# mgholamikn/PoseGen

Measured on AMD Instinct MI355X. Metric: rendered rays/sec (512x512, 64 samples/ray), higher is better.
Workload: dtype bf16

## Files before the change

include/posegen_hip.h:

```cpp
#ifndef POSEGEN_HIP_H
#define POSEGEN_HIP_H

#include <stdint.h>

#ifdef __cplusplus
extern "C" {
#endif

#define PG_ABI_VERSION 11

#define PG_OK 0
#define PG_EINVAL (-1)
#define PG_ENOMEM (-2)
#define PG_EHIP (-3)
#define PG_ESTATE (-4)

#define PG_PREC_FP32 0
#define PG_PREC_BF16 1
#define PG_PREC_BF16X3 2
#define PG_PREC_FP16 3
#define PG_PREC_FP16X3 4
#define PG_PREC_FP16C 5
#define PG_PREC_COUNT 6
#define PG_PREC_FP16M 6
// ... 138 lines not shown

int pg_stage_eval(pg_handle* h, void* stream, int which_net, int64_t n, int n_samples,
                  const float* ray_batch, const float* z, const float* skts,
                  int64_t pose_stride, const float* cams, float* raw, float* dbg, int dbg_stage);

int pg_query_density(pg_handle* h, void* stream, int which_net, int64_t n_points, const float* pts,
                     const float* skts, float* raw);

int pg_stage_composite(pg_handle* h, void* stream, int64_t n, int n_samples,
                       const float* ray_batch, const float* z, const float* raw,
                       float* rgb, float* disp, float* acc, float* alpha, float* weights,
                       int n_importance, float* z_fine );

int pg_set_far_skip(pg_handle* h, int on);

int pg_load_weights_device(pg_handle* h, void* stream, int which_net, const float* const* d_tensors, int n_tensors,
                           const float* d_codes, int n_codes);

#define PG_ONCHIP_RECORDS 0
#define PG_ONCHIP_AUTO 1
#define PG_ONCHIP_ALWAYS 2
int pg_set_onchip(pg_handle* h, int mode);

int pg_set_train_precision(pg_handle* h, int precision);

int pg_profile_enable(pg_handle* h, int on);
int pg_profile_read(pg_handle* h, int64_t* n_launches, double* total_ms, int64_t* n_points);
int pg_profile_read_aux(pg_handle* h, int64_t* n_launches, double* total_ms);

int pg_debug_pack(const float* const* tensors, const int64_t* shapes, int n_tensors,
// ... 24 lines not shown
```

posegen_amd/_ffi.py:

```python
from __future__ import annotations

import ctypes as C
import os
from typing import Optional

_HERE = os.path.dirname(os.path.abspath(__file__))
LIB_PATH = os.path.join(_HERE, "_lib", "libposegen_hip.so")

PG_OK, PG_EINVAL, PG_ENOMEM, PG_EHIP, PG_ESTATE = 0, -1, -2, -3, -4
PG_FLAG_LINDISP = 1
PG_ACT_RELU, PG_ACT_SOFTPLUS = 0, 1
PG_ABI_VERSION = 11


class HipLibraryError(RuntimeError):
    """libposegen_hip.so is missing or unusable (no CPU fallback exists)."""


class PgError(RuntimeError):
    def __init__(self, code: int, msg: str):
        super().__init__(f"posegen_hip error {code}: {msg}")
        self.code = code


# ... 26 lines not shown
                                   "alpha0", "near_far", "z_coarse", "z_fine", "raw_coarse", "raw_fine",
                                   "weights0")]


PROTOTYPES = {
    "pg_abi_version": (C.c_int, []),
    "pg_create": (C.c_int, [C.POINTER(PgConfig), C.c_int, C.POINTER(C.c_int), C.POINTER(C.c_void_p)]),
    "pg_destroy": (None, [C.c_void_p]),
    "pg_last_error": (C.c_char_p, [C.c_void_p]),
    "pg_load_weights": (C.c_int, [C.c_void_p, C.c_int, C.POINTER(C.c_void_p), C.POINTER(C.c_int64), C.c_int]),
    "pg_set_embedder": (C.c_int, [C.c_void_p, C.c_int, C.c_void_p, C.c_float]),
    "pg_set_framecodes": (C.c_int, [C.c_void_p, C.c_int, C.c_void_p, C.c_int]),
    "pg_set_precision": (C.c_int, [C.c_void_p, C.c_int]),
    "pg_set_chunk": (C.c_int, [C.c_void_p, C.c_int]),
    "pg_set_far_skip": (C.c_int, [C.c_void_p, C.c_int]),
    "pg_set_onchip": (C.c_int, [C.c_void_p, C.c_int]),
    "pg_load_weights_device": (C.c_int, [C.c_void_p, C.c_void_p, C.c_int, C.POINTER(C.c_void_p), C.c_int, C.c_void_p, C.c_int]),
    "pg_set_train_precision": (C.c_int, [C.c_void_p, C.c_int]),
    "pg_render_rays": (C.c_int, [C.c_void_p, C.c_void_p, C.c_int64, _FP, _FP, C.c_int64, _FP, C.c_int64, _FP,
                                 C.c_int, C.c_int, C.c_int, C.POINTER(PgOutputs)]),
    "pg_calibrate_mfma": (C.c_int, [C.c_void_p, C.c_int, C.c_int, C.c_double, C.POINTER(C.c_double), C.POINTER(C.c_double)]),
    "pg_render_rays_train": (C.c_int, [C.c_void_p, C.c_void_p, C.c_int64, _FP, _FP, C.c_int64, _FP, C.c_int64, _FP,
                                       C.c_int, C.c_int, C.c_int, C.POINTER(PgTrainDraws), C.POINTER(PgOutputs)]),
    "pg_stage_sample_coarse": (C.c_int, [C.c_void_p, C.c_void_p, C.c_int64, _FP, _FP, C.c_int64, C.c_int,
                                         C.c_int, _FP, _FP]),
    "pg_stage_eval": (C.c_int, [C.c_void_p, C.c_void_p, C.c_int, C.c_int64, C.c_int, _FP, _FP, _FP,
                                C.c_int64, _FP, _FP, _FP, C.c_int]),
    "pg_stage_composite": (C.c_int, [C.c_void_p, C.c_void_p, C.c_int64, C.c_int, _FP, _FP, _FP, _FP, _FP, _FP,
                                     _FP, _FP, C.c_int, _FP]),
    "pg_profile_enable": (C.c_int, [C.c_void_p, C.c_int]),
# ... 75 lines not shown
```

posegen_amd/csrc/pg_api.hip:

```cpp
#include <hip/hip_runtime.h>

#include <cstdarg>
#include <cstdio>
#include <cstdlib>
#include <chrono>
#include <cstring>
#include <algorithm>
#include <mutex>
#include <thread>
#include <new>
#include <utility>
#include <vector>

#include "../../include/posegen_hip.h"
#include "pg_device.h"
#include "pg_handle.h"
#include "pg_pack.h"

extern "C" {
int pg_launch_eval16(const pgd::EvalArgs* a, int fp16, int framecode, int grid, void* stream);
int pg_launch_eval16r(const pgd::EvalArgs* a, int fp16, int framecode, int onchip, int grid, void* stream);
int pg_launch_ray_records(const pgd::RecArgs* a, int fp16, int framecode, int n_cu, void* stream);
int pg_eval16_points_per_pass(void);
int pg_eval16_wgs_per_cu(void);
// ... 137 lines not shown
    F_C2,
    F_COMP_DIRECT,
    F_COMP_REC,
    F_COMP_ONCHIP,
    F_KMAJOR,
    F_COUNT
};

constexpr int PASS_WALK_RHO = 99;
struct Switches {
    bool view_fact = true;
    bool comp_kernel = true;
    bool comp_rec = true;
    bool evalc2 = true;
    int onchip = PG_ONCHIP_AUTO;
    int pass_walk = PASS_WALK_RHO;
};
const Switches& switches() {
    static const Switches sw = [] {
        auto off = [](const char* name) { const char* e = std::getenv(name); return e && e[0] == '0'; };
        Switches s;
        s.view_fact = !off("POSEGEN_VIEW_FACT");
        s.comp_kernel = !off("POSEGEN_COMP_KERNEL");
        s.comp_rec = !off("POSEGEN_COMP_REC");
        s.evalc2 = !off("POSEGEN_EVALC2");
        const char* e = std::getenv("POSEGEN_ONCHIP");
        s.onchip = e && e[0] == '0' ? PG_ONCHIP_RECORDS : e && e[0] == '2' ? PG_ONCHIP_ALWAYS : PG_ONCHIP_AUTO;
        if (const char* w = std::getenv("POSEGEN_PASS_WALK")) s.pass_walk = std::max(0, std::atoi(w));
        return s;
    }();
    return sw;
}

struct CallFacts {
    int prec;
    int S;
    long long pose_stride;
    bool fc;
    bool points, pnoise;
    bool dbg; int dbg_stage;
// ... 227 lines not shown
    hipError_t e = hipMalloc(reinterpret_cast<void**>(&h->ws), want);
    if (e != hipSuccess) return pg_fail(h, PG_ENOMEM, "workspace allocation of %zu bytes failed: %s", want, hipGetErrorString(e));
    h->ws_bytes = want;
    return PG_OK;
}

int check_ready(pg_handle* h, bool need_fine) {
    if (!h) return pg_fail(nullptr, PG_EINVAL, "null handle");
    need_fine = need_fine && !h->cfg.single_net;
    if (!h->net[0].loaded) return pg_fail(h, PG_ESTATE, "coarse network weights not loaded (pg_load_weights)");
    if (need_fine && !h->net[1].loaded) return pg_fail(h, PG_ESTATE, "fine network weights not loaded (pg_load_weights)");
    if (!h->emb_set[0] || !h->emb_set[1]) return pg_fail(h, PG_ESTATE, "embedder state not set (pg_set_embedder)");
    return PG_OK;
}

int launch_eval_one(pg_handle* h, void* stream, int which, long long n, int S, const float* rays, const float* z,
                    const float* skts, long long pose_stride, const float* cams, float* raw, float* dbg, int dbg_stage,
                    const float* points, const float* pnoise, bool guide_pass) {
    const int prec = pass_precision(h->cfg.precision, guide_pass);
    const bool fc = h->cfg.framecode_ch > 0;
    const Form form = pick_form(CallFacts{prec, S, pose_stride, fc, points != nullptr, pnoise != nullptr, dbg != nullptr, dbg_stage, h->onchip_mode}, switches());
    const FormInfo& fi = FORMS[form];
    const int y_bytes = fi.rec_y_bytes;
    int rc = ensure_form_images(h, which, form, prec, fc);
    if (rc) return rc;
    if (y_bytes && (rc = ensure_rec(h, n, y_bytes))) return rc;
    NetState& ns = h->net[which];
    if (fc && !ns.d_codes) return pg_fail(h, PG_ESTATE, "frame codes of net %d not set (pg_set_framecodes)", which);
    pgd::EvalArgs a{};
    a.rays = rays; a.z = z; a.pts = points; a.pnoise = pnoise; a.skts = skts; a.cams = cams;
    a.codes = fc ? ns.d_codes : nullptr;
    a.wstream = ns.img[image_of(fi.stream, prec)].d;
    a.wy = fi.wy == IMG_NONE || (fi.wy == IMG_YCODE && !fc) ? nullptr : ns.img[image_of(fi.wy, prec)].d;
    a.bias = reinterpret_cast<const float*>(ns.img[fi.bias].d);
    if (y_bytes) {
        a.rec_y = h->rec;
// ... 4 lines not shown
                                     (size_t)REC_PAD_RAYS * REC_AB_BYTES, static_cast<hipStream_t>(stream)));
            h->rec_pad_n = n; h->rec_pad_y = y_bytes; h->rec_pad_stream = stream;
        }
    }
    a.cutoff = h->d_cut;
    a.raw = raw; a.dbg = dbg;
    a.pose_stride = pose_stride;
    a.n_points = n * S;
    a.n_rays = (int)n;
    a.S = S;
    a.n_codes = ns.n_codes;
    a.tau_v = h->tau[0];
    a.tau_d = h->tau[1];
    a.dbg_stage = dbg_stage;
    a.far_skip = h->far_skip ? 1 : 0;
    const int pts = fi.points_per_pass();
    if (!points && S < pts / (MAXR - 1))
        return pg_fail(h, PG_EINVAL, "N_samples=%d too small: the fused kernel needs >= %d samples per ray", S, pts / (MAXR - 1));
    const long long iters = (a.n_points + pts - 1) / pts;
    a.n_iters = (int)iters;
    static const long long wg_cap = [] { const char* e = std::getenv("POSEGEN_MAX_WG"); return e ? std::atoll(e) : 0ll; }();
    long long max_wg = (long long)h->n_cu * fi.wgs_per_cu();
    if (wg_cap > 0 && wg_cap < max_wg) max_wg = wg_cap;
    const int grid = (int)(iters < max_wg ? iters : max_wg);
    a.walk_rho = switches().pass_walk % grid;
    hipEvent_t e0 = nullptr, e1 = nullptr;
    auto get = [&](hipEvent_t& ev) {
        if (!h->ev_free.empty()) { ev = h->ev_free.back(); h->ev_free.pop_back(); return hipSuccess; }
        return hipEventCreate(&ev);
    };
// ... 28 lines not shown
    case F_COMP_REC:    e = pg_launch_evalc(&a, fc, 1, grid, stream); break;
    case F_COMP_ONCHIP: e = pg_launch_evalc(&a, fc, 2, grid, stream); break;
    default:            e = pg_launch_eval32(&a, prec, fc, grid, stream); break;
    }
    if (h->profiling) {
        PG_HIP(h, hipEventRecord(e1, static_cast<hipStream_t>(stream)));
        h->ev_used.emplace_back(e0, e1);
        h->prof_points += a.n_points;
    }
    if (e) return pg_fail(h, PG_EHIP, "fused embed+MLP kernel launch failed: %s", hipGetErrorString((hipError_t)e));
    return PG_OK;
}

int launch_eval(pg_handle* h, void* stream, int which, long long n, int S, const float* rays, const float* z,
                const float* skts, long long pose_stride, const float* cams, float* raw, float* dbg, int dbg_stage = 0,
                const float* points = nullptr, const float* pnoise = nullptr, bool guide_pass = false) {
    long long batch = 1ll << 19;
    if (const char* e = std::getenv("POSEGEN_REC_BATCH")) { const long long v = std::atoll(e); if (v >= 64) batch = v; }
    if (points || dbg || n <= batch)
        return launch_eval_one(h, stream, which, n, S, rays, z, skts, pose_stride, cams, raw, dbg, dbg_stage, points, pnoise, guide_pass);
    for (long long r0 = 0; r0 < n; r0 += batch) {
        const long long m = std::min(batch, n - r0);
        const int rc = launch_eval_one(h, stream, which, m, S, rays + r0 * 11, z + r0 * S, skts + r0 * pose_stride, pose_stride,
                                       cams ? cams + r0 : nullptr, raw + r0 * S * 4, nullptr, 0, nullptr,
                                       pnoise ? pnoise + r0 * S * 3 : nullptr, guide_pass);
        if (rc) return rc;
    }
    return PG_OK;
}

}

int pg_sc_scratch(pg_handle* h, long long n, int chunk, double** out) {
    *out = nullptr;
    const long long need = pg_sample_coarse_scratch(n, chunk);
    if (need <= 0) return PG_OK;
    if ((size_t)need > h->sc_part_cap) {
        PG_HIP(h, hipSetDevice(h->device));
        if (h->sc_part) { PG_HIP(h, hipDeviceSynchronize()); PG_HIP(h, hipFree(h->sc_part)); h->sc_part = nullptr; h->sc_part_cap = 0; }
        const size_t want = (size_t)need * 2;
// ... 19 lines not shown
    if (cfg->n_joints != J || cfg->multires != LV || (cfg->multires_views != LD && cfg->multires_views != 0) || cfg->multires_bones != 0 ||
        cfg->net_depth != DEPTH || cfg->net_width != W || cfg->skip_layer != SKIP || cfg->view_width != VW ||
        (cfg->framecode_ch != 0 && cfg->framecode_ch != FC_CH))
        return pg_fail(nullptr, PG_EINVAL,
                    "pg_create: unsupported architecture (kernels are built for 24 joints, multires 7/{4,0}/0, "
                    "8x256 trunk, skip 4, view width 128, frame code 0|16)");
    if (cfg->single_net != 0 && cfg->single_net != 1) return pg_fail(nullptr, PG_EINVAL, "pg_create: single_net must be 0 or 1, got %d", cfg->single_net);
    if (cfg->precision < 0 || cfg->precision >= PG_PREC_MODES) return pg_fail(nullptr, PG_EINVAL, "pg_create: bad precision %d", cfg->precision);
    if (is_x3(cfg->precision) && !x3_allowed())
        return pg_fail(nullptr, PG_EINVAL, "pg_create: split-operand precision %d is experimental (set POSEGEN_EXPERIMENTAL_X3=1)", cfg->precision);
    if (cfg->chunk <= 0) return pg_fail(nullptr, PG_EINVAL, "pg_create: chunk must be positive");
    if (!(cfg->density_scale > 0.f)) return pg_fail(nullptr, PG_EINVAL, "pg_create: density_scale must be positive");
    if (cfg->density_act != PG_ACT_RELU && cfg->density_act != PG_ACT_SOFTPLUS)
        return pg_fail(nullptr, PG_EINVAL, "pg_create: density_act must be PG_ACT_RELU or PG_ACT_SOFTPLUS, got %d", cfg->density_act);
    pg_handle* h = new (std::nothrow) pg_handle();
    if (h) h->onchip_mode = switches().onchip;
    if (!h) return pg_fail(nullptr, PG_ENOMEM, "pg_create: out of host memory");
    h->cfg = *cfg;
    h->device = device_ids ? device_ids[0] : 0;
    for (int i = 0; i < 48; ++i) h->cut[i] = cfg->cutoff_dist;
    int ndev = 0;
    hipError_t e = hipGetDeviceCount(&ndev);
    if (e != hipSuccess || ndev <= 0) { delete h; return pg_fail(nullptr, PG_EHIP, "pg_create: no HIP device available (%s)", hipGetErrorString(e)); }
    if (h->device < 0 || h->device >= ndev) { delete h; return pg_fail(nullptr, PG_EINVAL, "pg_create: device %d out of range (%d devices)", cfg ? device_ids ? device_ids[0] : 0 : 0, ndev); }
    hipDeviceProp_t prop;
    if (hipSetDevice(h->device) != hipSuccess || hipGetDeviceProperties(&prop, h->device) != hipSuccess) {
        delete h;
        return pg_fail(nullptr, PG_EHIP, "pg_create: cannot query device");
    }
    h->n_cu = prop.multiProcessorCount > 0 ? prop.multiProcessorCount : 256;
    h->clock_khz = prop.clockRate;
// ... 223 lines not shown
    return PG_OK;
}

int pg_set_chunk(pg_handle* h, int chunk) {
    if (!h) return pg_fail(nullptr, PG_EINVAL, "pg_set_chunk: null handle");
    if (chunk <= 0) return pg_fail(h, PG_EINVAL, "pg_set_chunk: chunk must be positive, got %d", chunk);
    h->cfg.chunk = chunk;
    PG_FORWARD(h, pg_set_chunk(hh, chunk));
    return PG_OK;
}

int pg_set_far_skip(pg_handle* h, int on) {
    if (!h) return pg_fail(nullptr, PG_EINVAL, "pg_set_far_skip: null handle");
    h->far_skip = on != 0;
    PG_FORWARD(h, pg_set_far_skip(hh, on));
    return PG_OK;
}

int pg_set_onchip(pg_handle* h, int mode) {
    if (!h) return pg_fail(nullptr, PG_EINVAL, "pg_set_onchip: null handle");
    if (mode < PG_ONCHIP_RECORDS || mode > PG_ONCHIP_ALWAYS) return pg_fail(h, PG_EINVAL, "pg_set_onchip: mode must be 0 (records), 1 (by sample count) or 2 (on chip), got %d", mode);
    h->onchip_mode = mode;
    PG_FORWARD(h, pg_set_onchip(hh, mode));
    return PG_OK;
}

int pg_set_train_precision(pg_handle* h, int precision) {
    if (!h) return pg_fail(nullptr, PG_EINVAL, "null handle");
    if (precision != PG_PREC_FP32 && precision != PG_PREC_BF16)
        return pg_fail(h, PG_EINVAL, "pg_set_train_precision: the training step computes in fp32 (PG_PREC_FP32) or on a bf16 tape (PG_PREC_BF16), not %d", precision);
// ... 248 lines not shown
    if (e) return pg_fail(h, PG_EHIP, "sample_coarse launch failed: %s", hipGetErrorString((hipError_t)e));
    return PG_OK;
}

int pg_stage_eval(pg_handle* h, void* stream, int which, int64_t n, int n_samples, const float* ray_batch,
                  const float* z, const float* skts, int64_t pose_stride, const float* cams, float* raw, float* dbg,
                  int dbg_stage) {
    int rc = check_ready(h, which == 1);
    if (rc) return rc;
    if (which < 0 || which > 1) return pg_fail(h, PG_EINVAL, "pg_stage_eval: which_net must be 0 or 1");
    if (which == 1 && h->cfg.single_net) return pg_fail(h, PG_EINVAL, "pg_stage_eval: a single_net handle has one net (which_net 0)");
    if (n < 0 || !ray_batch || !z || !skts || !raw) return pg_fail(h, PG_EINVAL, "pg_stage_eval: null/negative argument");
    if (pose_stride != 0 && pose_stride != 384) return pg_fail(h, PG_EINVAL, "pose_stride must be 0 or 384");
    if (n == 0) return PG_OK;
    PG_HIP(h, hipSetDevice(h->device));
    return launch_eval(h, stream, which, n, n_samples, ray_batch, z, skts, pose_stride, cams, raw, dbg, dbg_stage);
}

int pg_query_density(pg_handle* h, void* stream, int which, int64_t n_points, const float* pts, const float* skts,
                     float* raw) {
    int rc = check_ready(h, which == 1);
    if (rc) return rc;
    if (which < 0 || which > 1) return pg_fail(h, PG_EINVAL, "pg_query_density: which_net must be 0 or 1");
    if (which == 1 && h->cfg.single_net) return pg_fail(h, PG_EINVAL, "pg_query_density: a single_net handle has one net (which_net 0)");
    if (n_points < 0 || !pts || !skts || !raw) return pg_fail(h, PG_EINVAL, "pg_query_density: null/negative argument");
    if (n_points > 0x7fffffffLL) return pg_fail(h, PG_EINVAL, "pg_query_density: at most 2^31-1 points per call");
    if (n_points == 0) return PG_OK;
    PG_HIP(h, hipSetDevice(h->device));
    rc = ensure_ws(h, 256);
    if (rc) return rc;
    PG_HIP(h, hipMemsetAsync(h->ws, 0, 64, static_cast<hipStream_t>(stream)));
// ... 67 lines not shown
    int* order = reinterpret_cast<int*>(p); p += b_ord;
    float* zn = reinterpret_cast<float*>(p); p += b_zn;
    float* rawn = reinterpret_cast<float*>(p); p += b_rn;
    float* pn = b_pn ? reinterpret_cast<float*>(p) : nullptr;
    {
        double* scs = nullptr;
        if (int rc2 = pg_sc_scratch(h, n, h->cfg.chunk, &scs)) return rc2;
        int e0 = pg_launch_sample_coarse(ray_batch, cyls, cyl_stride, n, h->cfg.chunk, S, (flags & PG_FLAG_LINDISP) ? 1 : 0, nf, zc,
                                         dr ? dr->t_rand : nullptr, scs, stream);
        if (e0) return pg_fail(h, PG_EHIP, "coarse sampling launch failed: %s", hipGetErrorString((hipError_t)e0));
    }
    if (rnoise) {
        int e0 = pg_launch_gather_noise(dr->ray_noise, n, SF, S, nullptr, pn, stream);
        if (e0) return pg_fail(h, PG_EHIP, "noise gather launch failed: %s", hipGetErrorString((hipError_t)e0));
    }
    rc = launch_eval(h, stream, 0, n, S, ray_batch, zc, skts, pose_stride, cams, rawc, nullptr, 0, nullptr, rnoise ? pn : nullptr, false);
    if (rc) return rc;
    int e = pg_launch_composite_iso(ray_batch, zc, rawc, n, S, h->cfg.density_scale, h->cfg.rgb_eps, h->cfg.density_act,
                                    h->cfg.softplus_shift, out->rgb0, out->disp0, out->acc0, out->alpha0,
                                    out->weights0 ? out->weights0 : w0, N, zf, dr ? dr->noise0 : nullptr, dr ? dr->u_rand : nullptr,
                                    order, zn, NP, stream);
    if (e) return pg_fail(h, PG_EHIP, "composite launch failed: %s", hipGetErrorString((hipError_t)e));
    if (rnoise) {
        e = NP == N ? pg_launch_gather_noise(dr->ray_noise + (size_t)S * 3, n, SF, N, nullptr, pn, stream)
                    : (int)hipMemsetAsync(pn, 0, (size_t)n * NP * 12, s);
        if (!e && NP != N)
            e = (int)hipMemcpy2DAsync(pn, (size_t)NP * 12, dr->ray_noise + (size_t)S * 3, (size_t)SF * 12, (size_t)N * 12, (size_t)n,
                                      hipMemcpyDeviceToDevice, s);
        if (e) return pg_fail(h, PG_EHIP, "noise gather failed: %s", hipGetErrorString((hipError_t)e));
    }
    rc = launch_eval(h, stream, 0, n, NP, ray_batch, zn, skts, pose_stride, cams, rawn, nullptr, 0, nullptr, rnoise ? pn : nullptr, false);
    if (rc) return rc;
    e = pg_launch_composite_merged(ray_batch, zf, rawc, rawn, NP, order, n, S, N, h->cfg.density_scale, h->cfg.rgb_eps, h->cfg.density_act,
                                   h->cfg.softplus_shift, out->rgb_map, out->disp_map, out->acc_map, out->alpha,
                                   dr ? dr->noise1 : nullptr, out->raw_fine, stream);
    if (e) return pg_fail(h, PG_EHIP, "composite launch failed: %s", hipGetErrorString((hipError_t)e));
    if (out->near_far) PG_HIP(h, hipMemcpyAsync(out->near_far, nf, (size_t)n * 8, hipMemcpyDeviceToDevice, s));
    if (out->z_coarse) PG_HIP(h, hipMemcpyAsync(out->z_coarse, zc, (size_t)n * S * 4, hipMemcpyDeviceToDevice, s));
    if (out->raw_coarse) PG_HIP(h, hipMemcpyAsync(out->raw_coarse, rawc, (size_t)n * S * 16, hipMemcpyDeviceToDevice, s));
    if (out->z_fine) PG_HIP(h, hipMemcpyAsync(out->z_fine, zf, (size_t)n * SF * 4, hipMemcpyDeviceToDevice, s));
    return PG_OK;
}

int render_rays_impl(pg_handle* h, void* stream, int64_t n, const float* ray_batch, const float* skts,
                     int64_t pose_stride, const float* cyls, int64_t cyl_stride, const float* cams, int n_samples,
                     int n_importance, int flags, const pg_train_draws* dr, const pg_outputs* out) {
// ... 30 lines not shown
    float* rawf = reinterpret_cast<float*>(p); p += hier ? b_rf : 0;
    int* order = b_ord ? reinterpret_cast<int*>(p) : nullptr; p += b_ord;
    float* pn = b_pn ? reinterpret_cast<float*>(p) : nullptr;

    {
        double* scs = nullptr;
        if (int rc = pg_sc_scratch(h, n, h->cfg.chunk, &scs)) return rc;
        int e0 = pg_launch_sample_coarse(ray_batch, cyls, cyl_stride, n, h->cfg.chunk, S, (flags & PG_FLAG_LINDISP) ? 1 : 0, nf, zc,
                                         dr ? dr->t_rand : nullptr, scs, stream);
        if (e0) return pg_fail(h, PG_EHIP, "coarse sampling launch failed: %s", hipGetErrorString((hipError_t)e0));
    }
    if (rnoise) {
        int e0 = pg_launch_gather_noise(dr->ray_noise, n, SF, S, nullptr, pn, stream);
        if (e0) return pg_fail(h, PG_EHIP, "noise gather launch failed: %s", hipGetErrorString((hipError_t)e0));
    }
    rc = launch_eval(h, stream, 0, n, S, ray_batch, zc, skts, pose_stride, cams, rawc, nullptr, 0, nullptr, rnoise ? pn : nullptr, hier);
    if (rc) return rc;
    int e = pg_launch_composite(ray_batch, zc, rawc, n, S, h->cfg.density_scale, h->cfg.rgb_eps, h->cfg.density_act, h->cfg.softplus_shift,
                                hier ? out->rgb0 : out->rgb_map, hier ? out->disp0 : out->disp_map,
                                hier ? out->acc0 : out->acc_map, hier ? out->alpha0 : out->alpha,
                                out->weights0 ? out->weights0 : w0, n_importance, hier ? zf : nullptr,
                                dr ? dr->noise0 : nullptr, dr ? dr->u_rand : nullptr, order, stream);
    if (e) return pg_fail(h, PG_EHIP, "composite launch failed: %s", hipGetErrorString((hipError_t)e));
    if (hier) {
        if (rnoise) {
            e = pg_launch_gather_noise(dr->ray_noise, n, SF, SF, order, pn, stream);
            if (e) return pg_fail(h, PG_EHIP, "noise gather launch failed: %s", hipGetErrorString((hipError_t)e));
        }
        rc = launch_eval(h, stream, 1, n, SF, ray_batch, zf, skts, pose_stride, cams, rawf, nullptr, 0, nullptr, rnoise ? pn : nullptr);
        if (rc) return rc;
        e = pg_launch_composite(ray_batch, zf, rawf, n, SF, h->cfg.density_scale, h->cfg.rgb_eps, h->cfg.density_act, h->cfg.softplus_shift, out->rgb_map,
                                out->disp_map, out->acc_map, out->alpha, nullptr, 0, nullptr, dr ? dr->noise1 : nullptr,
                                nullptr, nullptr, stream);
        if (e) return pg_fail(h, PG_EHIP, "composite launch failed: %s", hipGetErrorString((hipError_t)e));
    }
    if (out->near_far) PG_HIP(h, hipMemcpyAsync(out->near_far, nf, (size_t)n * 8, hipMemcpyDeviceToDevice, s));
    if (out->z_coarse) PG_HIP(h, hipMemcpyAsync(out->z_coarse, zc, (size_t)n * S * 4, hipMemcpyDeviceToDevice, s));
    if (out->raw_coarse) PG_HIP(h, hipMemcpyAsync(out->raw_coarse, rawc, (size_t)n * S * 16, hipMemcpyDeviceToDevice, s));
    if (hier && out->z_fine) PG_HIP(h, hipMemcpyAsync(out->z_fine, zf, (size_t)n * SF * 4, hipMemcpyDeviceToDevice, s));
    if (hier && out->raw_fine) PG_HIP(h, hipMemcpyAsync(out->raw_fine, rawf, (size_t)n * SF * 16, hipMemcpyDeviceToDevice, s));
    return PG_OK;
}
}

// ... 500 lines not shown
```

posegen_amd/csrc/pg_device.h:

```cpp
#pragma once
#include <hip/hip_runtime.h>

#include <atomic>

#include "pg_program.h"

namespace pgd {
using namespace pgl;

typedef __attribute__((ext_vector_type(8))) __bf16 bf16x8;
typedef __attribute__((ext_vector_type(8))) _Float16 f16x8;
typedef __attribute__((ext_vector_type(16))) float f32x16;

struct EvalArgs {
    const float* rays;
    const float* z;
    const float* pts;
    const float* pnoise;
    const float* skts;
    const float* cams;
    const float* codes;
    const uint8_t* wstream;
    const uint8_t* wy;
    const float* rec_ab;
    const uint8_t* rec_y;
    const float* bias;
    const float* cutoff;
    float* raw;
    float* dbg;
    long long pose_stride;
    long long n_points;
    int n_rays;
    int S;
    int n_codes;
    int n_iters;
    float tau_v, tau_d;
    int dbg_stage;
    int far_skip;
    int walk_rho;
};

struct RecArgs {
    const float* rays;
    const float* skts;
    const float* cams;
    const float* codes;
    const uint8_t* wy;
    float* rec_ab;
    uint8_t* rec_y;
    const float* z;
    long long pose_stride;
    int n_rays;
    int n_codes;
// ... 433 lines not shown
```

posegen_amd/csrc/pg_eval16_common.h:

```cpp
#pragma once
#include "pg_device.h"

namespace pgd {
using namespace pgp::A;

#ifndef PG_A_WAVES
#define PG_A_WAVES 8
#endif
constexpr int NWAVE = PG_A_WAVES;
constexpr int NTHR = NWAVE * 64;
constexpr int PTS = NWAVE * 32;

template <typename V> struct Op;
template <> struct Op<bf16x8> {
    using E = __bf16;
    static __device__ __forceinline__ f32x16 mfma(bf16x8 a, bf16x8 b, f32x16 c) {
#if defined(PG_MFMA_TURNS)
        asm volatile("s_setprio 1\n\tv_mfma_f32_32x32x16_bf16 %0, %1, %2, %0\n\ts_setprio 0" : "+v"(c) : "v"(a), "v"(b));
        return c;
#endif
        return __builtin_amdgcn_mfma_f32_32x32x16_bf16(a, b, c, 0, 0, 0);
    }
    static __device__ __forceinline__ bf16x8 cvt(const float* x) {
        bf16x8 v;
// ... 111 lines not shown
    }
#endif
    if (LA <= rem) st.issue(p.r[(L + LA) % NS], q + LA);
    if (PG_SPREAD_DMA) {
        if (q % PSTRIDE == PG_DMA_PHASE) st.piece(q / PSTRIDE);
        if (L == T - 1)
            for (int i = (q < PG_DMA_PHASE ? 0 : (q - PG_DMA_PHASE) / PSTRIDE + 1); i < PER; ++i) st.piece(i);
    }
    if (PG_EARLY_RETIRE) {
        if (q == 0) lds_retire(p.r[L % NS], min(LA, rem));
        if (rem >= 1) lds_retire(p.r[(L + 1) % NS], min(LA, rem) - 1);
    } else {
        lds_retire(p.r[L % NS], min(LA, rem));
    }
    return __builtin_bit_cast(V, p.r[L % NS]);
}

__device__ __forceinline__ void lds_async128(a128& dst, unsigned lds_addr) {
    asm volatile("ds_read_b128 %0, %1 offset:0+0" : "=v"(dst) : "v"(lds_addr));
}
__device__ __forceinline__ void lds_landed(a128& r) { asm volatile("" : "+v"(r)); }
__device__ __forceinline__ unsigned lds_addr_of(const void* p) {
    return (unsigned)(uintptr_t)(const __attribute__((address_space(3))) void*)p;
}

template <typename V, int T, int NS, int Q0, typename ST>
__device__ __forceinline__ V next_a_cont(APipe<V, NS>& p, ST& st, int L) {
    static_assert(Q0 + T <= UPC, "a continuation stays inside its chunk");
    constexpr int LA = NS - 1;
    const int q = Q0 + L, rem = T - 1 - L;
// ... 168 lines not shown
```

posegen_amd/csrc/pg_eval16r.hip:

```cpp
#ifndef PG_PREFETCH
#define PG_PREFETCH 1
#endif
#ifndef PG_PIPE_H
#define PG_PIPE_H 4
#endif
#include <type_traits>

#include "pg_eval16_common.h"

#ifndef PG_REC_POLICY
#define PG_REC_POLICY ""
#endif

namespace pgd {

typedef __attribute__((ext_vector_type(4))) float f32x4;

template <typename V> struct Op16;
template <> struct Op16<bf16x8> {
    static __device__ __forceinline__ f32x4 mfma(bf16x8 a, bf16x8 b, f32x4 c) {
        return __builtin_amdgcn_mfma_f32_16x16x32_bf16(a, b, c, 0, 0, 0);
    }
};
template <> struct Op16<f16x8> {
// ... 481 lines not shown
#pragma unroll
                for (int c = 0; c < 2; ++c) fb[u][c] = relu_pack16<V>(acc[2 * u][c], acc[2 * u + 1][c], true);
        }
        PG_STAMP(4);
        hidden_layer16<V>(fb, fa, st, bbase, BS_LAYER0 + 6 * NT16, C_L6);
        hidden_layer16<V>(fa, fb, st, bbase, BS_LAYER0 + 7 * NT16, C_L6 + CH);
        PG_STAMP(5);
        int gmask_n = 0;
#if !defined(PG_NO_FAR_SKIP)
        gmask_n = pass_far_mask(smem + LDSR_AB + (abuf ^ 1) * LDS_AB_BYTES, rays_of_pass(pw.p0n, off0n),
                                opaque_ptr(cut + 2 * J + JG * g_p), g_p, lane_p & 15);
        if (!a.far_skip) gmask_n = 0;
#endif
        st.nx_mask = (uint32_t)gmask_n;
        float sigma[2];
        V fg[NTV16 / 2][2];
        APipe<V> pv;
        {
            f32x4 vacc[NTV16][2];
            constexpr int TAV = pgp::R::U_AV;
            static_assert(BS_VIEWF == BS_ALPHA + 1 && BS_RGB == BS_VIEWF + NTV16, "alpha, view and rgb bias tiles are consecutive");
            BiasPipe bp(bbase, BS_ALPHA);
            bp.fetch(0);
#pragma unroll
            for (int o = 0; o < NTV16 + 1; ++o) {
                f32x4 t0, t1;
#pragma unroll
                for (int u = 0; u < HU16; ++u) {
                    const V av = next_a<V, TAV, true, PG_PIPE_H>(pv, st, o * HU16 + u, C_AV);
                    if (u == 0) t0 = t1 = bp.take();
                    t0 = Op16<V>::mfma(av, fb[u][0], t0);
                    t1 = Op16<V>::mfma(av, fb[u][1], t1);
                    if (u == PG_R_BIAS_AT && o < NTV16) bp.fetch(o + 1);
                }
                if (o == 0) { sigma[0] = t0[0]; sigma[1] = t1[0]; }
                else { vacc[o - 1][0] = t0; vacc[o - 1][1] = t1; }
            }
            PG_STAMP(6);
            float wd[2][JG];
#pragma unroll
            for (int jj = 0; jj < JG; ++jj) {
                float qx, qy, qz;
                q0(jj, qx, qy, qz);
                wd[0][jj] = cutoff_weight_fast(__builtin_amdgcn_sqrtf(qx * qx + qy * qy + qz * qz), tld, cutd[jj]);
                q1(jj, qx, qy, qz);
                wd[1][jj] = cutoff_weight_fast(__builtin_amdgcn_sqrtf(qx * qx + qy * qy + qz * qz), tld, cutd[jj]);
                if (OC && ((gmask >> jj) & 1)) wd[0][jj] = wd[1][jj] = 0.0f;
            }
            y_apply16<V, FC>(vacc, smem + LDSR_Y, wd, myr, lane_p);
#pragma unroll
            for (int u = 0; u < NTV16 / 2; ++u)
#pragma unroll
                for (int c = 0; c < 2; ++c) fg[u][c] = relu_pack16<V>(vacc[2 * u][c], vacc[2 * u + 1][c], true);
        }
        PG_STAMP(7);
        PG_PREFETCH_Z(itn);
        f32x4 c0, c1;
        {
            APipe<V> pr;
            BiasPipe bp(bbase, BS_RGB);
            bp.fetch(0);
#pragma unroll
            for (int u = 0; u < pgp::R::U_RGB; ++u) {
                const V av = next_a_cont<V, pgp::R::U_RGB, PG_PIPE_H, pgp::R::U_AV % UPC>(pr, st, u);
                if (u == 0) c0 = c1 = bp.take();
                c0 = Op16<V>::mfma(av, fg[u][0], c0);
                c1 = Op16<V>::mfma(av, fg[u][1], c1);
            }
        }
        if (g == 0) {
            const int i = wave * 32 + col;
            if (i <= last) *reinterpret_cast<float4*>(a.raw + (p0 + i) * 4) = make_float4(c0[0], c0[1], c0[2], sigma[0]);
            if (i + 16 <= last) *reinterpret_cast<float4*>(a.raw + (p0 + i + 16) * 4) = make_float4(c1[0], c1[1], c1[2], sigma[1]);
        }
        abuf ^= 1;
        pw.advance(); pw.peek();
        p0 = pw.p0; r0 = pw.r0; off0 = pw.off0;
        gmask = gmask_n;
        PG_STAMP(8);
#if defined(PG_STAMPS)
        if (a.dbg && a.dbg_stage == 99 && lane == 0 && it < 64) {
            for (int k = 0; k < 9; ++k) reinterpret_cast<unsigned long long*>(a.dbg)[((long long)it * NWAVE + wave) * 16 + k] = stamps[k];
// ... 53 lines not shown
```

posegen_amd/csrc/pg_handle.h:

```cpp
#pragma once
#include <hip/hip_runtime.h>

#include <utility>
#include <vector>

#include "../../include/posegen_hip.h"
#include "pg_layout.h"

enum Image : int {
    IMG_NONE = -1,
    IMG_DIRECT = 0,
    IMG_REC16 = IMG_DIRECT + PG_PREC_COUNT,
    IMG_ONCHIP16 = IMG_REC16 + PG_PREC_COUNT,
    IMG_VY16 = IMG_ONCHIP16 + PG_PREC_COUNT,
    IMG_PER_PREC_END = IMG_VY16 + PG_PREC_COUNT,
    IMG_COMP_DIRECT = IMG_PER_PREC_END,
    IMG_COMP_REC,
    IMG_VYC,
    IMG_COMP_ONCHIP,
    IMG_C2,
    IMG_YCODE,
    IMG_BIAS16,
    IMG_BIAS,
    IMG_COUNT
// ... 29 lines not shown
    uint8_t* ws = nullptr;
    size_t ws_bytes = 0;
    uint8_t* fws = nullptr;
    size_t fws_bytes = 0;
    double* sc_part = nullptr;
    size_t sc_part_cap = 0;
    uint8_t* rec = nullptr;
    size_t rec_bytes = 0;
    long long rec_pad_n = -1;
    int rec_pad_y = 0;
    void* rec_pad_stream = nullptr;
    std::vector<pg_handle*> peers;
    hipStream_t own_stream = nullptr;
    float* d_pose = nullptr;
    bool far_skip = true;
    int onchip_mode = PG_ONCHIP_AUTO;
    int train_precision = PG_PREC_FP32;
    bool profiling = false;
    std::vector<hipEvent_t> ev_free;
    std::vector<std::pair<hipEvent_t, hipEvent_t>> ev_used;
    std::vector<std::pair<hipEvent_t, hipEvent_t>> ev_aux;
    int64_t aux_n = 0;
    double aux_ms = 0.0;
    int64_t prof_points = 0;
    void* train = nullptr;
    struct FramesCache {
        size_t hw = 0;
        bool has_u8 = false;
        static constexpr int NBUF = 2;
        float* d_frame[NBUF] = {};
// ... 26 lines not shown
```

posegen_amd/raycaster.py:

```python
from __future__ import annotations

import ctypes as C
from typing import Dict, Optional

import numpy as np
import torch

from . import _ffi
from .config import PREC_BF16, PREC_BY_NAME, PREC_NAMES, RenderConfig

NET_TENSOR_ORDER = ([f"pts_linears.{l}.{k}" for l in range(8) for k in ("weight", "bias")]
                    + [f"{n}.{k}" for n in ("alpha_linear", "feature_linear", "views_linears.0", "rgb_linear")
                       for k in ("weight", "bias")])


def _density_act(density_type: str) -> int:
    try:
        return {"relu": _ffi.PG_ACT_RELU, "softplus": _ffi.PG_ACT_SOFTPLUS}[density_type]
    except KeyError:
        raise NotImplementedError(f"density activation {density_type} is undefined") from None


def _np32(x) -> np.ndarray:
    if isinstance(x, torch.Tensor):
# ... 31 lines not shown
                           precision=self.precision, cutoff_dist=cfg.cutoff_dist,
                           density_scale=cfg.density_scale, rgb_eps=cfg.rgb_eps,
                           softplus_shift=float(cfg.softplus_shift), density_act=_density_act(cfg.density_type),
                           single_net=1 if cfg.single_net else 0)
        idx = self.device.index if self.device.index is not None else torch.cuda.current_device()
        dev_ids = [idx] if devices is None else devices
        ids = (C.c_int * len(dev_ids))(*dev_ids)
        self.devices = list(dev_ids)
        h = C.c_void_p()
        rc = self.lib.pg_create(C.byref(pc), len(dev_ids), ids, C.byref(h))
        _ffi.check(self.lib, None, rc)
        self.handle = h
        self._state: Dict[str, dict] = {}
        self._state_lazy: Dict[str, object] = {}
        self._chunk = cfg.chunk

    def close(self):
        if getattr(self, "handle", None):
            self.lib.pg_destroy(self.handle)
            self.handle = None

    def __del__(self):
        try:
            self.close()
        except Exception:
            pass

    def _check(self, rc):
        _ffi.check(self.lib, self.handle, rc)

# ... 52 lines not shown
        self.precision = int(precision)

    def set_chunk(self, chunk: int):
        if int(chunk) != self._chunk:
            self._check(self.lib.pg_set_chunk(self.handle, int(chunk)))
            self._chunk = int(chunk)

    def set_onchip(self, mode="auto"):
        modes = {"records": 0, "auto": 1, "always": 2, 0: 0, 1: 1, 2: 2}
        if mode not in modes:
            raise ValueError(f"set_onchip: mode must be 'records', 'auto' or 'always', not {mode!r}")
        self._check(self.lib.pg_set_onchip(self.handle, modes[mode]))

    def set_far_skip(self, on=True):
        self._check(self.lib.pg_set_far_skip(self.handle, 1 if on else 0))

    def set_train_precision(self, precision="fp32"):
        p = PREC_BY_NAME[precision] if isinstance(precision, str) else int(precision)
        self._check(self.lib.pg_set_train_precision(self.handle, p))

    def profile_enable(self, on=True):
        self._check(self.lib.pg_profile_enable(self.handle, 1 if on else 0))

    def profile_read(self):
        n, ms, pts = C.c_int64(), C.c_double(), C.c_int64()
        self._check(self.lib.pg_profile_read(self.handle, C.byref(n), C.byref(ms), C.byref(pts)))
        return n.value, ms.value, pts.value

    def profile_read_aux(self):
        n, ms = C.c_int64(), C.c_double()
# ... 302 lines not shown
        dbg = torch.zeros(n * S, 256, device=self.device) if want_dbg else None
        self._check(self.lib.pg_stage_eval(self.handle, self._stream(), int(which), n, S, _ptr(rb), _ptr(zz),
                                           _ptr(sk), ps, _ptr(cam), _ptr(raw), _ptr(dbg), int(dbg_stage)))
        return (raw, dbg) if want_dbg else raw

    def limb_skip_stats(self, which, ray_batch, z, skts, cams=None):
        rb = _dev_f32(ray_batch, self.device)
        zz = _dev_f32(z, self.device)
        n, S = zz.shape
        sk, ps = self._pose_args(skts, n)
        cam = None if cams is None else _dev_f32(cams.reshape(-1), self.device)
        raw = torch.empty(n, S, 4, device=self.device)
        cnt = torch.zeros(64, device=self.device, dtype=torch.int32)
        self._check(self.lib.pg_stage_eval(self.handle, self._stream(), int(which), n, S, _ptr(rb), _ptr(zz),
                                           _ptr(sk), ps, _ptr(cam), _ptr(raw), cnt.data_ptr(), 97))
        passes, per_pass, fine = (int(v) for v in cnt[:3].cpu())
        per_fine = 48
        return {"passes": passes, "limbs_left_out_of_whole_passes_frac": per_pass / max(6 * passes, 1),
                "limbs_left_out_frac": fine / max(per_fine * passes, 1)}

    def stage_composite(self, ray_batch, z, raw, n_importance=0):
        rb = _dev_f32(ray_batch, self.device)
        zz = _dev_f32(z, self.device)
        rw = _dev_f32(raw, self.device)
        n, S = zz.shape
        new = lambda *s: torch.empty(*s, device=self.device, dtype=torch.float32)
        o = {"rgb_map": new(n, 3), "disp_map": new(n), "acc_map": new(n), "alpha": new(n, S),
             "weights": new(n, S)}
        zf = new(n, S + n_importance) if n_importance > 0 else None
        self._check(self.lib.pg_stage_composite(self.handle, self._stream(), n, S, _ptr(rb), _ptr(zz), _ptr(rw),
                                                _ptr(o["rgb_map"]), _ptr(o["disp_map"]), _ptr(o["acc_map"]),
                                                _ptr(o["alpha"]), _ptr(o["weights"]), int(n_importance), _ptr(zf)))
        if zf is not None:
            o["z_fine"] = zf
        return o


def _same_state(a, b) -> bool:
    if set(a) != set(b):
        return False
    return all(np.array_equal(_np32(a[k]), _np32(b[k])) for k in a)


class HipRayCaster:

    def __init__(self, cfg: RenderConfig, device="cuda:0", precision=PREC_BF16, devices=None):
        self.cfg = cfg
        self.renderer = HipRenderer(cfg, device, precision, devices=devices)
        self.training = False

# ... 214 lines not shown
```

Baseline: 8.743 million.

## Skip view and RGB heads for waves whose samples all have zero density

```diff
diff --git a/include/posegen_hip.h b/include/posegen_hip.h
--- a/include/posegen_hip.h
+++ b/include/posegen_hip.h
@@ -176,6 +176,10 @@
 
 int pg_set_far_skip(pg_handle* h, int on);
 
+int pg_set_empty_skip(pg_handle* h, int on);
+
+int pg_debug_wave_counts(pg_handle* h, uint32_t* counts);
+
 int pg_load_weights_device(pg_handle* h, void* stream, int which_net, const float* const* d_tensors, int n_tensors,
                            const float* d_codes, int n_codes);
 
diff --git a/posegen_amd/_ffi.py b/posegen_amd/_ffi.py
--- a/posegen_amd/_ffi.py
+++ b/posegen_amd/_ffi.py
@@ -64,6 +64,8 @@
     "pg_set_precision": (C.c_int, [C.c_void_p, C.c_int]),
     "pg_set_chunk": (C.c_int, [C.c_void_p, C.c_int]),
     "pg_set_far_skip": (C.c_int, [C.c_void_p, C.c_int]),
+    "pg_set_empty_skip": (C.c_int, [C.c_void_p, C.c_int]),
+    "pg_debug_wave_counts": (C.c_int, [C.c_void_p, C.c_void_p]),
     "pg_set_onchip": (C.c_int, [C.c_void_p, C.c_int]),
     "pg_load_weights_device": (C.c_int, [C.c_void_p, C.c_void_p, C.c_int, C.POINTER(C.c_void_p), C.c_int, C.c_void_p, C.c_int]),
     "pg_set_train_precision": (C.c_int, [C.c_void_p, C.c_int]),
diff --git a/posegen_amd/csrc/pg_api.hip b/posegen_amd/csrc/pg_api.hip
--- a/posegen_amd/csrc/pg_api.hip
+++ b/posegen_amd/csrc/pg_api.hip
@@ -175,6 +175,7 @@
     bool comp_rec = true;
     bool evalc2 = true;
     int onchip = PG_ONCHIP_AUTO;
+    bool empty_skip = true;
     int pass_walk = PASS_WALK_RHO;
 };
 const Switches& switches() {
@@ -185,6 +186,7 @@
         s.comp_kernel = !off("POSEGEN_COMP_KERNEL");
         s.comp_rec = !off("POSEGEN_COMP_REC");
         s.evalc2 = !off("POSEGEN_EVALC2");
+        s.empty_skip = !off("POSEGEN_EMPTY_SKIP");
         const char* e = std::getenv("POSEGEN_ONCHIP");
         s.onchip = e && e[0] == '0' ? PG_ONCHIP_RECORDS : e && e[0] == '2' ? PG_ONCHIP_ALWAYS : PG_ONCHIP_AUTO;
         if (const char* w = std::getenv("POSEGEN_PASS_WALK")) s.pass_walk = std::max(0, std::atoi(w));
@@ -442,12 +444,17 @@
     return PG_OK;
 }
 
+bool skip_empty_ok(const pg_handle* h, bool colour_free) {
+    return colour_free && h->empty_skip && h->cfg.density_act == PG_ACT_RELU && h->cfg.density_scale > 0.0f;
+}
+
 int launch_eval_one(pg_handle* h, void* stream, int which, long long n, int S, const float* rays, const float* z,
                     const float* skts, long long pose_stride, const float* cams, float* raw, float* dbg, int dbg_stage,
-                    const float* points, const float* pnoise, bool guide_pass) {
+                    const float* points, const float* pnoise, bool guide_pass, bool colour_free) {
     const int prec = pass_precision(h->cfg.precision, guide_pass);
     const bool fc = h->cfg.framecode_ch > 0;
-    const Form form = pick_form(CallFacts{prec, S, pose_stride, fc, points != nullptr, pnoise != nullptr, dbg != nullptr, dbg_stage, h->onchip_mode}, switches());
+    Form form = pick_form(CallFacts{prec, S, pose_stride, fc, points != nullptr, pnoise != nullptr, dbg != nullptr, dbg_stage, h->onchip_mode}, switches());
+    if (!dbg && h->wave_counts && form == F_ONCHIP16 && pose_stride == 0 && !fc) { dbg = reinterpret_cast<float*>(h->wave_counts); dbg_stage = 97; }
     const FormInfo& fi = FORMS[form];
     const int y_bytes = fi.rec_y_bytes;
     int rc = ensure_form_images(h, which, form, prec, fc);
@@ -482,6 +489,7 @@
     a.tau_d = h->tau[1];
     a.dbg_stage = dbg_stage;
     a.far_skip = h->far_skip ? 1 : 0;
+    a.skip_empty = skip_empty_ok(h, colour_free) ? 1 : 0;
     const int pts = fi.points_per_pass();
     if (!points && S < pts / (MAXR - 1))
         return pg_fail(h, PG_EINVAL, "N_samples=%d too small: the fused kernel needs >= %d samples per ray", S, pts / (MAXR - 1));
@@ -540,16 +548,16 @@
 
 int launch_eval(pg_handle* h, void* stream, int which, long long n, int S, const float* rays, const float* z,
                 const float* skts, long long pose_stride, const float* cams, float* raw, float* dbg, int dbg_stage = 0,
-                const float* points = nullptr, const float* pnoise = nullptr, bool guide_pass = false) {
+                const float* points = nullptr, const float* pnoise = nullptr, bool guide_pass = false, bool colour_free = false) {
     long long batch = 1ll << 19;
     if (const char* e = std::getenv("POSEGEN_REC_BATCH")) { const long long v = std::atoll(e); if (v >= 64) batch = v; }
     if (points || dbg || n <= batch)
-        return launch_eval_one(h, stream, which, n, S, rays, z, skts, pose_stride, cams, raw, dbg, dbg_stage, points, pnoise, guide_pass);
+        return launch_eval_one(h, stream, which, n, S, rays, z, skts, pose_stride, cams, raw, dbg, dbg_stage, points, pnoise, guide_pass, colour_free);
     for (long long r0 = 0; r0 < n; r0 += batch) {
         const long long m = std::min(batch, n - r0);
         const int rc = launch_eval_one(h, stream, which, m, S, rays + r0 * 11, z + r0 * S, skts + r0 * pose_stride, pose_stride,
                                        cams ? cams + r0 : nullptr, raw + r0 * S * 4, nullptr, 0, nullptr,
-                                       pnoise ? pnoise + r0 * S * 3 : nullptr, guide_pass);
+                                       pnoise ? pnoise + r0 * S * 3 : nullptr, guide_pass, colour_free);
         if (rc) return rc;
     }
     return PG_OK;
@@ -599,7 +607,7 @@
     if (cfg->density_act != PG_ACT_RELU && cfg->density_act != PG_ACT_SOFTPLUS)
         return pg_fail(nullptr, PG_EINVAL, "pg_create: density_act must be PG_ACT_RELU or PG_ACT_SOFTPLUS, got %d", cfg->density_act);
     pg_handle* h = new (std::nothrow) pg_handle();
-    if (h) h->onchip_mode = switches().onchip;
+    if (h) { h->onchip_mode = switches().onchip; h->empty_skip = switches().empty_skip; }
     if (!h) return pg_fail(nullptr, PG_ENOMEM, "pg_create: out of host memory");
     h->cfg = *cfg;
     h->device = device_ids ? device_ids[0] : 0;
@@ -853,6 +861,19 @@
     if (!h) return pg_fail(nullptr, PG_EINVAL, "pg_set_far_skip: null handle");
     h->far_skip = on != 0;
     PG_FORWARD(h, pg_set_far_skip(hh, on));
+    return PG_OK;
+}
+
+int pg_set_empty_skip(pg_handle* h, int on) {
+    if (!h) return pg_fail(nullptr, PG_EINVAL, "pg_set_empty_skip: null handle");
+    h->empty_skip = on != 0;
+    PG_FORWARD(h, pg_set_empty_skip(hh, on));
+    return PG_OK;
+}
+
+int pg_debug_wave_counts(pg_handle* h, uint32_t* counts) {
+    if (!h) return pg_fail(nullptr, PG_EINVAL, "pg_debug_wave_counts: null handle");
+    h->wave_counts = counts;
     return PG_OK;
 }
 
@@ -1131,7 +1152,8 @@
     if (pose_stride != 0 && pose_stride != 384) return pg_fail(h, PG_EINVAL, "pose_stride must be 0 or 384");
     if (n == 0) return PG_OK;
     PG_HIP(h, hipSetDevice(h->device));
-    return launch_eval(h, stream, which, n, n_samples, ray_batch, z, skts, pose_stride, cams, raw, dbg, dbg_stage);
+    return launch_eval(h, stream, which, n, n_samples, ray_batch, z, skts, pose_stride, cams, raw, dbg, dbg_stage, nullptr, nullptr, false,
+                       dbg && dbg_stage == 97);
 }
 
 int pg_query_density(pg_handle* h, void* stream, int which, int64_t n_points, const float* pts, const float* skts,
@@ -1229,7 +1251,9 @@
         int e0 = pg_launch_gather_noise(dr->ray_noise, n, SF, S, nullptr, pn, stream);
         if (e0) return pg_fail(h, PG_EHIP, "noise gather launch failed: %s", hipGetErrorString((hipError_t)e0));
     }
-    rc = launch_eval(h, stream, 0, n, S, ray_batch, zc, skts, pose_stride, cams, rawc, nullptr, 0, nullptr, rnoise ? pn : nullptr, false);
+    const bool free_c = !out->raw_coarse && !out->raw_fine && !(dr && (dr->noise0 || dr->noise1));
+    const bool free_n = !out->raw_fine && !(dr && dr->noise1);
+    rc = launch_eval(h, stream, 0, n, S, ray_batch, zc, skts, pose_stride, cams, rawc, nullptr, 0, nullptr, rnoise ? pn : nullptr, false, free_c);
     if (rc) return rc;
     int e = pg_launch_composite_iso(ray_batch, zc, rawc, n, S, h->cfg.density_scale, h->cfg.rgb_eps, h->cfg.density_act,
                                     h->cfg.softplus_shift, out->rgb0, out->disp0, out->acc0, out->alpha0,
@@ -1244,7 +1268,7 @@
                                       hipMemcpyDeviceToDevice, s);
         if (e) return pg_fail(h, PG_EHIP, "noise gather failed: %s", hipGetErrorString((hipError_t)e));
     }
-    rc = launch_eval(h, stream, 0, n, NP, ray_batch, zn, skts, pose_stride, cams, rawn, nullptr, 0, nullptr, rnoise ? pn : nullptr, false);
+    rc = launch_eval(h, stream, 0, n, NP, ray_batch, zn, skts, pose_stride, cams, rawn, nullptr, 0, nullptr, rnoise ? pn : nullptr, false, free_n);
     if (rc) return rc;
     e = pg_launch_composite_merged(ray_batch, zf, rawc, rawn, NP, order, n, S, N, h->cfg.density_scale, h->cfg.rgb_eps, h->cfg.density_act,
                                    h->cfg.softplus_shift, out->rgb_map, out->disp_map, out->acc_map, out->alpha,
@@ -1305,7 +1329,9 @@
         int e0 = pg_launch_gather_noise(dr->ray_noise, n, SF, S, nullptr, pn, stream);
         if (e0) return pg_fail(h, PG_EHIP, "noise gather launch failed: %s", hipGetErrorString((hipError_t)e0));
     }
-    rc = launch_eval(h, stream, 0, n, S, ray_batch, zc, skts, pose_stride, cams, rawc, nullptr, 0, nullptr, rnoise ? pn : nullptr, hier);
+    const bool free_c = !out->raw_coarse && !(dr && dr->noise0);
+    const bool free_f = !out->raw_fine && !(dr && dr->noise1);
+    rc = launch_eval(h, stream, 0, n, S, ray_batch, zc, skts, pose_stride, cams, rawc, nullptr, 0, nullptr, rnoise ? pn : nullptr, hier, free_c);
     if (rc) return rc;
     int e = pg_launch_composite(ray_batch, zc, rawc, n, S, h->cfg.density_scale, h->cfg.rgb_eps, h->cfg.density_act, h->cfg.softplus_shift,
                                 hier ? out->rgb0 : out->rgb_map, hier ? out->disp0 : out->disp_map,
@@ -1318,7 +1344,7 @@
             e = pg_launch_gather_noise(dr->ray_noise, n, SF, SF, order, pn, stream);
             if (e) return pg_fail(h, PG_EHIP, "noise gather launch failed: %s", hipGetErrorString((hipError_t)e));
         }
-        rc = launch_eval(h, stream, 1, n, SF, ray_batch, zf, skts, pose_stride, cams, rawf, nullptr, 0, nullptr, rnoise ? pn : nullptr);
+        rc = launch_eval(h, stream, 1, n, SF, ray_batch, zf, skts, pose_stride, cams, rawf, nullptr, 0, nullptr, rnoise ? pn : nullptr, false, free_f);
         if (rc) return rc;
         e = pg_launch_composite(ray_batch, zf, rawf, n, SF, h->cfg.density_scale, h->cfg.rgb_eps, h->cfg.density_act, h->cfg.softplus_shift, out->rgb_map,
                                 out->disp_map, out->acc_map, out->alpha, nullptr, 0, nullptr, dr ? dr->noise1 : nullptr,
diff --git a/posegen_amd/csrc/pg_device.h b/posegen_amd/csrc/pg_device.h
--- a/posegen_amd/csrc/pg_device.h
+++ b/posegen_amd/csrc/pg_device.h
@@ -37,6 +37,7 @@
     float tau_v, tau_d;
     int dbg_stage;
     int far_skip;
+    int skip_empty;
     int walk_rho;
 };
 
diff --git a/posegen_amd/csrc/pg_eval16_common.h b/posegen_amd/csrc/pg_eval16_common.h
--- a/posegen_amd/csrc/pg_eval16_common.h
+++ b/posegen_amd/csrc/pg_eval16_common.h
@@ -149,6 +149,20 @@
         lds_retire(p.r[L % NS], min(LA, rem));
     }
     return __builtin_bit_cast(V, p.r[L % NS]);
+}
+
+template <int T, int L0, typename ST>
+__device__ __forceinline__ void skip_units(ST& st, int c0 = -1) {
+    static_assert(PG_SPREAD_DMA, "the bulk enter() refills by itself");
+    constexpr int PER = ST::PER, PSTRIDE = UPC / PER;
+#pragma unroll
+    for (int L = L0; L < T; ++L) {
+        const int q = L % UPC;
+        if (q == 0) st.enter_split(c0 >= 0 && ST::plain_ok(c0 + L / UPC));
+        if (q % PSTRIDE == PG_DMA_PHASE) st.piece(q / PSTRIDE);
+        if (L == T - 1)
+            for (int i = (q < PG_DMA_PHASE ? 0 : (q - PG_DMA_PHASE) / PSTRIDE + 1); i < PER; ++i) st.piece(i);
+    }
 }
 
 __device__ __forceinline__ void lds_async128(a128& dst, unsigned lds_addr) {
diff --git a/posegen_amd/csrc/pg_eval16r.hip b/posegen_amd/csrc/pg_eval16r.hip
--- a/posegen_amd/csrc/pg_eval16r.hip
+++ b/posegen_amd/csrc/pg_eval16r.hip
@@ -519,17 +519,14 @@
 #endif
         st.nx_mask = (uint32_t)gmask_n;
         float sigma[2];
-        V fg[NTV16 / 2][2];
-        APipe<V> pv;
+        f32x4 c0, c1;
         {
-            f32x4 vacc[NTV16][2];
+            APipe<V> pv;
             constexpr int TAV = pgp::R::U_AV;
             static_assert(BS_VIEWF == BS_ALPHA + 1 && BS_RGB == BS_VIEWF + NTV16, "alpha, view and rgb bias tiles are consecutive");
             BiasPipe bp(bbase, BS_ALPHA);
             bp.fetch(0);
-#pragma unroll
-            for (int o = 0; o < NTV16 + 1; ++o) {
-                f32x4 t0, t1;
+            auto av_tile = [&](int o, f32x4& t0, f32x4& t1) __attribute__((always_inline)) {
 #pragma unroll
                 for (int u = 0; u < HU16; ++u) {
                     const V av = next_a<V, TAV, true, PG_PIPE_H>(pv, st, o * HU16 + u, C_AV);
@@ -538,39 +535,63 @@
                     t1 = Op16<V>::mfma(av, fb[u][1], t1);
                     if (u == PG_R_BIAS_AT && o < NTV16) bp.fetch(o + 1);
                 }
-                if (o == 0) { sigma[0] = t0[0]; sigma[1] = t1[0]; }
-                else { vacc[o - 1][0] = t0; vacc[o - 1][1] = t1; }
-            }
-            PG_STAMP(6);
-            float wd[2][JG];
-#pragma unroll
-            for (int jj = 0; jj < JG; ++jj) {
-                float qx, qy, qz;
-                q0(jj, qx, qy, qz);
-                wd[0][jj] = cutoff_weight_fast(__builtin_amdgcn_sqrtf(qx * qx + qy * qy + qz * qz), tld, cutd[jj]);
-                q1(jj, qx, qy, qz);
-                wd[1][jj] = cutoff_weight_fast(__builtin_amdgcn_sqrtf(qx * qx + qy * qy + qz * qz), tld, cutd[jj]);
-                if (OC && ((gmask >> jj) & 1)) wd[0][jj] = wd[1][jj] = 0.0f;
-            }
-            y_apply16<V, FC>(vacc, smem + LDSR_Y, wd, myr, lane_p);
-#pragma unroll
-            for (int u = 0; u < NTV16 / 2; ++u)
-#pragma unroll
-                for (int c = 0; c < 2; ++c) fg[u][c] = relu_pack16<V>(vacc[2 * u][c], vacc[2 * u + 1][c], true);
-        }
-        PG_STAMP(7);
-        PG_PREFETCH_Z(itn);
-        f32x4 c0, c1;
-        {
-            APipe<V> pr;
-            BiasPipe bp(bbase, BS_RGB);
-            bp.fetch(0);
-#pragma unroll
-            for (int u = 0; u < pgp::R::U_RGB; ++u) {
-                const V av = next_a_cont<V, pgp::R::U_RGB, PG_PIPE_H, pgp::R::U_AV % UPC>(pr, st, u);
-                if (u == 0) c0 = c1 = bp.take();
-                c0 = Op16<V>::mfma(av, fg[u][0], c0);
-                c1 = Op16<V>::mfma(av, fg[u][1], c1);
+            };
+            {
+                f32x4 t0, t1;
+                av_tile(0, t0, t1);
+                sigma[0] = t0[0]; sigma[1] = t1[0];
+            }
+            bool empty = false;
+            if (CNT || a.skip_empty) {
+                const int i = wave * 32 + (lane_p & 15);
+                const bool live = g_p == 0 && ((i <= last && !(sigma[0] <= 0.0f)) || (i + 16 <= last && !(sigma[1] <= 0.0f)));
+                empty = __builtin_amdgcn_ballot_w64(live) == 0ull;
+                if (CNT && lane == 0 && empty) {
+                    atomicAdd(reinterpret_cast<unsigned*>(a.dbg) + 3, 1u);
+                    if (a.skip_empty) atomicAdd(reinterpret_cast<unsigned*>(a.dbg) + 4, 1u);
+                }
+                empty = empty && a.skip_empty != 0;
+            }
+            if (empty) {
+                asm volatile("s_waitcnt lgkmcnt(0)" ::: "memory");
+                PG_STAMP(6);
+                skip_units<TAV, HU16>(st, C_AV);
+                PG_STAMP(7);
+                PG_PREFETCH_Z(itn);
+                c0 = c1 = f32x4{0.0f, 0.0f, 0.0f, 0.0f};
+            } else {
+                f32x4 vacc[NTV16][2];
+                V fg[NTV16 / 2][2];
+#pragma unroll
+                for (int o = 1; o < NTV16 + 1; ++o) av_tile(o, vacc[o - 1][0], vacc[o - 1][1]);
+                PG_STAMP(6);
+                float wd[2][JG];
+#pragma unroll
+                for (int jj = 0; jj < JG; ++jj) {
+                    float qx, qy, qz;
+                    q0(jj, qx, qy, qz);
+                    wd[0][jj] = cutoff_weight_fast(__builtin_amdgcn_sqrtf(qx * qx + qy * qy + qz * qz), tld, cutd[jj]);
+                    q1(jj, qx, qy, qz);
+                    wd[1][jj] = cutoff_weight_fast(__builtin_amdgcn_sqrtf(qx * qx + qy * qy + qz * qz), tld, cutd[jj]);
+                    if (OC && ((gmask >> jj) & 1)) wd[0][jj] = wd[1][jj] = 0.0f;
+                }
+                y_apply16<V, FC>(vacc, smem + LDSR_Y, wd, myr, lane_p);
+#pragma unroll
+                for (int u = 0; u < NTV16 / 2; ++u)
+#pragma unroll
+                    for (int c = 0; c < 2; ++c) fg[u][c] = relu_pack16<V>(vacc[2 * u][c], vacc[2 * u + 1][c], true);
+                PG_STAMP(7);
+                PG_PREFETCH_Z(itn);
+                APipe<V> pr;
+                BiasPipe bpr(bbase, BS_RGB);
+                bpr.fetch(0);
+#pragma unroll
+                for (int u = 0; u < pgp::R::U_RGB; ++u) {
+                    const V av = next_a_cont<V, pgp::R::U_RGB, PG_PIPE_H, pgp::R::U_AV % UPC>(pr, st, u);
+                    if (u == 0) c0 = c1 = bpr.take();
+                    c0 = Op16<V>::mfma(av, fg[u][0], c0);
+                    c1 = Op16<V>::mfma(av, fg[u][1], c1);
+                }
             }
         }
         if (g == 0) {
diff --git a/posegen_amd/csrc/pg_handle.h b/posegen_amd/csrc/pg_handle.h
--- a/posegen_amd/csrc/pg_handle.h
+++ b/posegen_amd/csrc/pg_handle.h
@@ -67,6 +67,8 @@
     hipStream_t own_stream = nullptr;
     float* d_pose = nullptr;
     bool far_skip = true;
+    bool empty_skip = true;
+    uint32_t* wave_counts = nullptr;
     int onchip_mode = PG_ONCHIP_AUTO;
     int train_precision = PG_PREC_FP32;
     bool profiling = false;
diff --git a/posegen_amd/raycaster.py b/posegen_amd/raycaster.py
--- a/posegen_amd/raycaster.py
+++ b/posegen_amd/raycaster.py
@@ -69,6 +69,7 @@
         self._state: Dict[str, dict] = {}
         self._state_lazy: Dict[str, object] = {}
         self._chunk = cfg.chunk
+        self._wave_counts = None
 
     def close(self):
         if getattr(self, "handle", None):
@@ -151,6 +152,18 @@
 
     def set_far_skip(self, on=True):
         self._check(self.lib.pg_set_far_skip(self.handle, 1 if on else 0))
+
+    def set_empty_skip(self, on=True):
+        self._check(self.lib.pg_set_empty_skip(self.handle, 1 if on else 0))
+
+    def count_waves(self, on=True):
+        self._wave_counts = torch.zeros(16, device=self.device, dtype=torch.int32) if on else None
+        self._check(self.lib.pg_debug_wave_counts(self.handle, self._wave_counts.data_ptr() if on else None))
+
+    def read_wave_counts(self):
+        c = [int(v) for v in self._wave_counts.cpu()]
+        self._wave_counts.zero_()
+        return _wave_stats(c)
 
     def set_train_precision(self, precision="fp32"):
         p = PREC_BY_NAME[precision] if isinstance(precision, str) else int(precision)
@@ -483,10 +496,7 @@
         cnt = torch.zeros(64, device=self.device, dtype=torch.int32)
         self._check(self.lib.pg_stage_eval(self.handle, self._stream(), int(which), n, S, _ptr(rb), _ptr(zz),
                                            _ptr(sk), ps, _ptr(cam), _ptr(raw), cnt.data_ptr(), 97))
-        passes, per_pass, fine = (int(v) for v in cnt[:3].cpu())
-        per_fine = 48
-        return {"passes": passes, "limbs_left_out_of_whole_passes_frac": per_pass / max(6 * passes, 1),
-                "limbs_left_out_frac": fine / max(per_fine * passes, 1)}
+        return _wave_stats([int(v) for v in cnt[:5].cpu()])
 
     def stage_composite(self, ray_batch, z, raw, n_importance=0):
         rb = _dev_f32(ray_batch, self.device)
@@ -503,6 +513,14 @@
         if zf is not None:
             o["z_fine"] = zf
         return o
+
+
+def _wave_stats(c):
+    passes, per_pass, fine, empty, skipped = c[:5]
+    per_fine = 48
+    return {"passes": passes, "limbs_left_out_of_whole_passes_frac": per_pass / max(6 * passes, 1),
+            "limbs_left_out_frac": fine / max(per_fine * passes, 1),
+            "empty_waves_frac": empty / max(8 * passes, 1), "skipped_waves_frac": skipped / max(8 * passes, 1)}
 
 
 def _same_state(a, b) -> bool:
```

Result: faster. 9.161 million, median of 6 (+4.8%).
